# darkAlert/sports-field-homography

Hardware: AMD Instinct MI355X
Metric: frames/sec at 640x360 batch=16 (1/2/4/8 GPU) + homography L1 vs ref (higher is better)
Workload: dtype f16x3->f32 (2-way fp16 split operands = 22 significand bits, 3 fp16 MFMA products, fp32 accumulate; end-to-end error at the level of an fp32 run, see DESIGN.md section 2); 1 GPU; predict(): UNet seg + ResNet34-STN + nearest warp, 640x360, batch 16/GPU, req_outputs=theta,warp_mask; global_batch=16, precision=f16x3, range_fallbacks=0, range_rescales=0, range_raises=0, parallelism=single GPU

## Files before the change

### sports-field-homography_amd/csrc/conv_upfused.hip

```cpp
#include "common.h"
#include "conv_epilogue.h"
#include "split_mfma.h"

namespace {

constexpr int TH = 16, TW = 32;
constexpr int LH = TH / 2 + 2, LW = TW / 2 + 2, LPIX = LH * LW, LPIXP = 192;
constexpr int SHH = TH + 2, SWW = TW + 2, SPIX = SHH * SWW, SPIXP = 624;
constexpr int LSLOTS = 8 * LPIXP, SSLOTS = 8 * SPIXP;

struct UpGeom {
  int tiles_y, tiles_x, ntiles, nblk;
  int xcd_order;
  unsigned bytes_skip, bytes_low;
};

__global__ __launch_bounds__(256, 2) void conv_upfused_kernel(const sfh_conv_desc d, const UpGeom g) {
  extern __shared__ __attribute__((aligned(16))) float smem_f[];
  u32x4* const lds = reinterpret_cast<u32x4*>(smem_f);
  typedef __attribute__((address_space(3))) void* lds_ptr_t;
  const int tid = threadIdx.x, lane = tid & 63, wv = __builtin_amdgcn_readfirstlane(tid >> 6);
  const int lq = lane & 15, lg = lane >> 4;
  const int py = wv >> 1, px = wv & 1, qd = wv;
  int nb, tile;
  if (g.xcd_order) {
    const SfhWg wg = sfh_wg_xcd_range_all((int)blockIdx.x & 7, (int)blockIdx.x >> 3, g.ntiles, g.nblk);
    if (!wg.live) return;
    nb = wg.nb;
    tile = wg.tile;
  } else {
    nb = (int)blockIdx.x % g.nblk;
    tile = (int)blockIdx.x / g.nblk;
  }
  const int tpi = g.tiles_y * g.tiles_x;
  const int b = tile / tpi, tr = tile - b * tpi;
  const int ty = tr / g.tiles_x;
  const int y0 = ty * TH, x0 = (tr - ty * g.tiles_x) * TW;
  const int Y0 = y0 >> 1, X0 = x0 >> 1;
  const int nst_low = d.c1 >> 5, nst_skip = d.c0 >> 5;
  const unsigned nblk_low = (unsigned)d.cs1 >> 5, nblk_skip = (unsigned)d.cs0 >> 5;
  const __amdgpu_buffer_rsrc_t r_skip = __builtin_amdgcn_make_buffer_rsrc(const_cast<float*>(d.src0), 0, (int)g.bytes_skip, 0x00020000);
  const __amdgpu_buffer_rsrc_t r_low = __builtin_amdgcn_make_buffer_rsrc(const_cast<float*>(d.src1), 0, (int)g.bytes_low, 0x00020000);
  using WS = SplitWeights<2>;
  const unsigned wtot_up = (unsigned)nst_low * 4u * WS::TAP, wtot_sk = (unsigned)nst_skip * 9u * WS::TAP;
  const __amdgpu_buffer_rsrc_t rw_up = __builtin_amdgcn_make_buffer_rsrc(
      const_cast<char*>(reinterpret_cast<const char*>(d.up_wpacked)) + (size_t)(qd * g.nblk + nb) * wtot_up, 0, (int)wtot_up, 0x00020000);
  const __amdgpu_buffer_rsrc_t rw_sk = __builtin_amdgcn_make_buffer_rsrc(
      const_cast<char*>(reinterpret_cast<const char*>(d.wpacked)) + (size_t)nb * wtot_sk, 0, (int)wtot_sk, 0x00020000);

  f32x4 acc[4][8];
#pragma unroll
  for (int n = 0; n < 4; ++n)
#pragma unroll
    for (int i = 0; i < 8; ++i) acc[n][i] = (f32x4){0.f, 0.f, 0.f, 0.f};

  auto run_phase = [&](auto ntap_tag, int nst, const __amdgpu_buffer_rsrc_t& rsrc, const __amdgpu_buffer_rsrc_t& rw,
                       auto&& halo_off, int nslots, int rowstride_bytes, auto&& xaddr) {
    constexpr int NTAP = decltype(ntap_tag)::value;
    constexpr int NSTEP = NTAP * 8;
    for (int st = 0; st < nst; ++st) {
      __syncthreads();
      const unsigned cb = (unsigned)st * (unsigned)rowstride_bytes;
      for (int s0 = tid; s0 < nslots; s0 += 256)
        __builtin_amdgcn_raw_ptr_buffer_load_lds(rsrc, (lds_ptr_t)(lds + (s0 - lane)), 16, (int)halo_off(s0), (int)cb, 0, 0);
      u32x4 wr[2][2][4], xq[3][2];
      auto ld_w = [&](int t, int set) {
#pragma unroll
        for (int p = 0; p < 2; ++p)
#pragma unroll
          for (int n = 0; n < 4; ++n)
            wr[set][p][n] = __builtin_bit_cast(u32x4, __builtin_amdgcn_raw_buffer_load_b128(
                rw, (int)((p * 4 + n) * WS::GROUP + lane * 16), (int)(((unsigned)st * NTAP + (unsigned)t) * WS::TAP), 0));
      };
      ld_w(0, 0);
      asm volatile("s_waitcnt vmcnt(8)" ::: "memory");
      __syncthreads();
      auto ld_x = [&](int s_, int set) {
        const int t = s_ >> 3, i = s_ & 7;
#pragma unroll
        for (int p = 0; p < 2; ++p) xq[set][p] = lds[xaddr(t, i, p)];
      };
      ld_x(0, 0);
      ld_x(1, 1);
#pragma unroll
      for (int s_ = 0; s_ < NSTEP; ++s_) {
        const int t = s_ >> 3, i = s_ & 7;
        if (s_ + 2 < NSTEP) ld_x(s_ + 2, (s_ + 2) % 3);
        if (i == 0 && t + 1 < NTAP) ld_w(t + 1, (t + 1) & 1);
        using P = SplitProducts<2>;
#pragma unroll
        for (int k = 0; k < P::N; ++k)
#pragma unroll
          for (int n = 0; n < 4; ++n) acc[n][i] = split_mfma<2>(wr[t & 1][P::PW[k]][n], xq[s_ % 3][P::PX[k]], acc[n][i]);
        __builtin_amdgcn_sched_group_barrier(0x008, 1, 0);
        if (s_ + 2 < NSTEP) __builtin_amdgcn_sched_group_barrier(0x100, 2, 0);
        if (i == 0 && t + 1 < NTAP) __builtin_amdgcn_sched_group_barrier(0x020, 8, 0);
        __builtin_amdgcn_sched_group_barrier(0x008, 11, 0);
        __builtin_amdgcn_sched_barrier(0);
      }
    }
  };

  {
    auto halo_off = [&](int slot) -> unsigned {
      const int plg = slot / LPIXP, p = slot - plg * LPIXP;
      const int hy = p / LW, hx = p - hy * LW;
      const int y = Y0 - 1 + hy, x = X0 - 1 + hx;
      const bool ok = p < LPIX && y >= 0 && y < d.h1 && x >= 0 && x < d.w1;
      return ok ? split_pixel_offset<2>((unsigned)(b * d.h1 + y), nblk_low, (unsigned)plg, (unsigned)d.w1, (unsigned)x) : kSfhOOB;
    };
    const int base = lg * LPIXP + py * LW + lq + px;
    auto xaddr = [&](int t, int i, int p) { return base + p * 4 * LPIXP + (i + (t >> 1)) * LW + (t & 1); };
    run_phase(std::integral_constant<int, 4>{}, nst_low, r_low, rw_up, halo_off, LSLOTS, 128 * d.w1, xaddr);
  }
  const int xo = x0 + 2 * lq + px;
  {
    const int uh = 2 * d.h1, uw = 2 * d.w1;
    const unsigned clsx = (unsigned)(xo == 0 ? 0 : (xo == uw - 1 ? 2 : (xo >= uw ? 3 : 1)));
#pragma unroll
    for (int i = 0; i < 8; ++i) {
      const int yo = y0 + 2 * i + py;
      const unsigned cls = (unsigned)(yo == 0 ? 0 : (yo == uh - 1 ? 2 : (yo >= uh ? 3 : 1))) * 4u + clsx;
#pragma unroll
      for (int n = 0; n < 4; ++n) {
        const int cov = qd * d.cout + nb * 64 + n * 16 + 4 * lg;
        const f32x4 sc = *reinterpret_cast<const f32x4*>(d.up_scale + cov);
        const f32x4 sh = *reinterpret_cast<const f32x4*>(d.shift_border + (size_t)cls * (size_t)(4 * d.cout) + cov);
#pragma unroll
        for (int j = 0; j < 4; ++j) acc[n][i][j] = acc[n][i][j] * sc[j] + sh[j];
      }
    }
  }
  {
    auto halo_off = [&](int slot) -> unsigned {
      const int plg = slot / SPIXP, p = slot - plg * SPIXP;
      const int hy = p / SWW, hx = p - hy * SWW;
      const int y = y0 - 1 + hy, x = x0 - 1 + hx;
      const bool ok = p < SPIX && y >= 0 && y < d.H && x >= 0 && x < d.W;
      return ok ? split_pixel_offset<2>((unsigned)(b * d.H + y), nblk_skip, (unsigned)plg, (unsigned)d.W, (unsigned)x) : kSfhOOB;
    };
    const int base = lg * SPIXP + py * SWW + 2 * lq + px;
    auto xaddr = [&](int t, int i, int p) { return base + p * 4 * SPIXP + (2 * i + t / 3) * SWW + (t % 3); };
    run_phase(std::integral_constant<int, 9>{}, nst_skip, r_skip, rw_sk, halo_off, SSLOTS, 128 * d.W, xaddr);
  }
  const float dscale = sfh_h2_pow2(d.h2_exp_dst);
  const unsigned cs = (unsigned)d.dst_cs, run = (unsigned)d.W * 16u, planeb = 4u * run;
  const __amdgpu_buffer_rsrc_t rd = __builtin_amdgcn_make_buffer_rsrc(d.dst, 0, (int)kSfhOOB, 0x00020000);
  unsigned over = 0u;
#pragma unroll
  for (int n = 0; n < 4; ++n) {
    const unsigned co = (unsigned)(nb * 64 + n * 16 + 4 * lg);
    const f32x4 sc = *reinterpret_cast<const f32x4*>(d.scale + co), sh = *reinterpret_cast<const f32x4*>(d.shift + co);
    const unsigned lane_co = ((co >> 5) * 8u + ((co & 31u) >> 3)) * run + ((co >> 2) & 1u) * 8u;
#pragma unroll
    for (int i = 0; i < 8; ++i) {
      f32x4 v = acc[n][i];
#pragma unroll
      for (int j = 0; j < 4; ++j) {
        v[j] = v[j] * sc[j] + sh[j];
        if (d.relu) v[j] = sfh_relu(v[j]);
      }
      const int yo = y0 + 2 * i + py;
      const bool ok = yo < d.H && xo < d.W;
      const unsigned voff = ok ? (unsigned)(b * d.H + yo) * ((cs >> 5) * 8u * run) + (unsigned)xo * 16u + lane_co : kSfhOOB;
      u32x2 pl[2];
      unsigned o = 0u;
      sfh_split4_h2(v, dscale, pl, o);
      o = ok ? o : 0u;
      over = o > over ? o : over;
#pragma unroll
      for (int p = 0; p < 2; ++p) __builtin_amdgcn_raw_buffer_store_b64(pl[p], rd, (int)voff, (int)(p * planeb), 0);
    }
  }
  sfh_h2_report(over, d.h2_overflow, d.h2_range);
}

}

extern "C" int sfh_conv_upfused_fwd(const sfh_conv_desc* dp, void* stream_) {
  SFH_REQUIRE(dp, "conv_upfused_fwd: null descriptor");
  const sfh_conv_desc& d = *dp;
  SFH_REQUIRE(d.src0 && d.src1 && d.wpacked && d.up_wpacked && d.up_scale && d.shift_border && d.scale && d.shift && d.dst,
              "conv_upfused_fwd: null pointer");
  SFH_REQUIRE(d.src_fmt == SFH_FMT_H2 && d.dst_fmt == SFH_FMT_H2, "conv_upfused_fwd: H2 sources and destination");
  SFH_REQUIRE(d.batch > 0 && d.H > 0 && d.W > 0 && d.h0 == d.H && d.w0 == d.W && d.h1 > 0 && d.w1 > 0 &&
                  (d.H == 2 * d.h1 || d.H == 2 * d.h1 + 1) && (d.W == 2 * d.w1 || d.W == 2 * d.w1 + 1),
              "conv_upfused_fwd: skip %dx%d against a low-resolution source %dx%d (twice its size, plus at most one padded row / column)",
              d.W, d.H, d.w1, d.h1);
  SFH_REQUIRE(d.cout > 0 && d.cout % 64 == 0 && d.c0 > 0 && d.c0 % 32 == 0 && d.cs0 >= d.c0 && d.cs0 % 32 == 0 && d.c1 > 0 &&
                  d.c1 % 32 == 0 && d.cs1 >= d.c1 && d.cs1 % 32 == 0 && d.dst_cs >= d.cout && d.dst_cs % 32 == 0,
              "conv_upfused_fwd: channel counts (cout %d, skip %d / %d, low %d / %d, dst %d)", d.cout, d.c0, d.cs0, d.c1, d.cs1, d.dst_cs);
  SFH_REQUIRE(!d.residual && !d.dst_pool && !d.head_w && !d.acc_init && !(d.ksplit > 1) && !d.stats_partial && !d.pool0,
              "conv_upfused_fwd: a plain launch (no residual / pooled output / head / acc_init / split-K / statistics)");
  if (!sfh_h2_exp_ok("conv_upfused_fwd", "h2_exp_dst", d.h2_exp_dst)) return SFH_E_ARG;
  UpGeom g;
  g.tiles_y = sfh_cdiv(d.H, TH);
  g.tiles_x = sfh_cdiv(d.W, TW);
  g.ntiles = d.batch * g.tiles_y * g.tiles_x;
  g.nblk = d.cout / 64;
  const unsigned long long bs = 4ULL * d.batch * d.H * d.W * d.cs0, bl = 4ULL * d.batch * d.h1 * d.w1 * d.cs1;
  SFH_REQUIRE(sfh_fits_descriptor(bs) && sfh_fits_descriptor(bl) && sfh_fits_descriptor(4ULL * d.batch * d.H * d.W * (unsigned long long)d.dst_cs),
              "conv_upfused_fwd: a tensor exceeds the 4 GiB descriptor range");
  g.bytes_skip = (unsigned)bs;
  g.bytes_low = (unsigned)bl;
  g.xcd_order = 1;
  const long nblocks = (long)sfh_cdiv(g.ntiles, 8) * 8 * g.nblk;
  SFH_REQUIRE(nblocks < (1L << 31), "conv_upfused_fwd: grid too large");
  sfh_allow_big_lds((const void*)conv_upfused_kernel);
  hipLaunchKernelGGL(conv_upfused_kernel, dim3((unsigned)nblocks), dim3(256), SSLOTS * 16, (hipStream_t)stream_, d, g);
  return sfh_check_launch("conv_upfused_kernel");
}
```

Measured before the change: 1275 frames/s.

## Tile upfused conv over batch-flattened rows with incremental halo address walk

Replaces per-image tiling with a grid that treats the batch as one stack of rows, so tiles can span image boundaries and fewer partial tiles are wasted at image edges. The halo staging loop now uses an incremental walker that advances coordinates per round instead of doing divisions per slot, and issues both split planes per iteration. The h2 range report is done with a wave-level max reduction and a single atomic per wave, skipping the atomic when the value is not above a pre-read range. This adds row-split logic per output row and depends on the new shared geometry helpers being correct.

```diff
diff --git a/sports-field-homography_amd/csrc/conv_upfused.hip b/sports-field-homography_amd/csrc/conv_upfused.hip
--- a/sports-field-homography_amd/csrc/conv_upfused.hip
+++ b/sports-field-homography_amd/csrc/conv_upfused.hip
@@ -1,16 +1,14 @@
 #include "common.h"
 #include "conv_epilogue.h"
 #include "split_mfma.h"
+#include "upfused_geom.h"
 
 namespace {
 
-constexpr int TH = 16, TW = 32;
-constexpr int LH = TH / 2 + 2, LW = TW / 2 + 2, LPIX = LH * LW, LPIXP = 192;
-constexpr int SHH = TH + 2, SWW = TW + 2, SPIX = SHH * SWW, SPIXP = 624;
-constexpr int LSLOTS = 8 * LPIXP, SSLOTS = 8 * SPIXP;
-
-struct UpGeom {
-  int tiles_y, tiles_x, ntiles, nblk;
+constexpr int LW = SfhUp::LW, LPIXP = SfhUp::LPIXP, SWW = SfhUp::SWW, SPIXP = SfhUp::SPIXP, SSLOTS = SfhUp::SSLOTS;
+
+struct UpGeom : SfhUpGrid {
+  int nblk;
   int xcd_order;
   unsigned bytes_skip, bytes_low;
 };
@@ -32,13 +30,10 @@
     nb = (int)blockIdx.x % g.nblk;
     tile = (int)blockIdx.x / g.nblk;
   }
-  const int tpi = g.tiles_y * g.tiles_x;
-  const int b = tile / tpi, tr = tile - b * tpi;
-  const int ty = tr / g.tiles_x;
-  const int y0 = ty * TH, x0 = (tr - ty * g.tiles_x) * TW;
-  const int Y0 = y0 >> 1, X0 = x0 >> 1;
+  int r0, x0;
+  sfh_up_tile_origin(g, tile, r0, x0);
+  const SfhUpSrc src_low{d.batch, d.h1, d.w1, (unsigned)d.cs1 >> 5}, src_skip{d.batch, d.H, d.W, (unsigned)d.cs0 >> 5};
   const int nst_low = d.c1 >> 5, nst_skip = d.c0 >> 5;
-  const unsigned nblk_low = (unsigned)d.cs1 >> 5, nblk_skip = (unsigned)d.cs0 >> 5;
   const __amdgpu_buffer_rsrc_t r_skip = __builtin_amdgcn_make_buffer_rsrc(const_cast<float*>(d.src0), 0, (int)g.bytes_skip, 0x00020000);
   const __amdgpu_buffer_rsrc_t r_low = __builtin_amdgcn_make_buffer_rsrc(const_cast<float*>(d.src1), 0, (int)g.bytes_low, 0x00020000);
   using WS = SplitWeights<2>;
@@ -54,15 +49,29 @@
 #pragma unroll
     for (int i = 0; i < 8; ++i) acc[n][i] = (f32x4){0.f, 0.f, 0.f, 0.f};
 
-  auto run_phase = [&](auto ntap_tag, int nst, const __amdgpu_buffer_rsrc_t& rsrc, const __amdgpu_buffer_rsrc_t& rw,
-                       auto&& halo_off, int nslots, int rowstride_bytes, auto&& xaddr) {
+  auto run_phase = [&](auto ntap_tag, auto walk_tag, auto low_tag, int nst, const __amdgpu_buffer_rsrc_t& rsrc,
+                       const __amdgpu_buffer_rsrc_t& rw, const SfhUpSrc& src, int rbase, int xbase, int rowstride_bytes,
+                       auto&& xaddr, auto&& before_last) {
     constexpr int NTAP = decltype(ntap_tag)::value;
     constexpr int NSTEP = NTAP * 8;
+    using Walk = decltype(walk_tag);
     for (int st = 0; st < nst; ++st) {
       __syncthreads();
+      if (st == nst - 1) before_last();
       const unsigned cb = (unsigned)st * (unsigned)rowstride_bytes;
-      for (int s0 = tid; s0 < nslots; s0 += 256)
-        __builtin_amdgcn_raw_ptr_buffer_load_lds(rsrc, (lds_ptr_t)(lds + (s0 - lane)), 16, (int)halo_off(s0), (int)cb, 0, 0);
+      Walk walk;
+      walk.start(tid);
+#pragma unroll 1
+      for (int k = 0; k < Walk::NROUND; ++k) {
+        const int w0 = k * SfhUp::NT + wv * 64;
+        const SfhUpOffsets off = sfh_up_halo_offsets<decltype(low_tag)::value>(g, src, rbase, xbase, walk);
+        if (w0 < Walk::PSLOTS) {
+#pragma unroll
+          for (int p = 0; p < 2; ++p)
+            __builtin_amdgcn_raw_ptr_buffer_load_lds(rsrc, (lds_ptr_t)(lds + (w0 + p * Walk::PSLOTS)), 16, (int)off.plane[p], (int)cb, 0, 0);
+        }
+        walk.step();
+      }
       u32x4 wr[2][2][4], xq[3][2];
       auto ld_w = [&](int t, int set) {
 #pragma unroll
@@ -102,25 +111,19 @@
   };
 
   {
-    auto halo_off = [&](int slot) -> unsigned {
-      const int plg = slot / LPIXP, p = slot - plg * LPIXP;
-      const int hy = p / LW, hx = p - hy * LW;
-      const int y = Y0 - 1 + hy, x = X0 - 1 + hx;
-      const bool ok = p < LPIX && y >= 0 && y < d.h1 && x >= 0 && x < d.w1;
-      return ok ? split_pixel_offset<2>((unsigned)(b * d.h1 + y), nblk_low, (unsigned)plg, (unsigned)d.w1, (unsigned)x) : kSfhOOB;
-    };
     const int base = lg * LPIXP + py * LW + lq + px;
     auto xaddr = [&](int t, int i, int p) { return base + p * 4 * LPIXP + (i + (t >> 1)) * LW + (t & 1); };
-    run_phase(std::integral_constant<int, 4>{}, nst_low, r_low, rw_up, halo_off, LSLOTS, 128 * d.w1, xaddr);
+    run_phase(std::integral_constant<int, 4>{}, SfhUpLowWalk{}, std::true_type{}, nst_low, r_low, rw_up, src_low,
+              sfh_up_low_row(r0) - 1, (x0 >> 1) - 1, 128 * d.w1, xaddr, [] {});
   }
   const int xo = x0 + 2 * lq + px;
   {
-    const int uh = 2 * d.h1, uw = 2 * d.w1;
-    const unsigned clsx = (unsigned)(xo == 0 ? 0 : (xo == uw - 1 ? 2 : (xo >= uw ? 3 : 1)));
+    const unsigned clsx = sfh_up_border_class(xo, 2 * d.w1);
 #pragma unroll
     for (int i = 0; i < 8; ++i) {
-      const int yo = y0 + 2 * i + py;
-      const unsigned cls = (unsigned)(yo == 0 ? 0 : (yo == uh - 1 ? 2 : (yo >= uh ? 3 : 1))) * 4u + clsx;
+      int ob, oy;
+      sfh_row_split(g, r0 + 2 * i + py, ob, oy);
+      const unsigned cls = sfh_up_border_class(oy, 2 * d.h1) * 4u + clsx;
 #pragma unroll
       for (int n = 0; n < 4; ++n) {
         const int cov = qd * d.cout + nb * 64 + n * 16 + 4 * lg;
@@ -131,17 +134,14 @@
       }
     }
   }
+  unsigned range_seen = 0u;
   {
-    auto halo_off = [&](int slot) -> unsigned {
-      const int plg = slot / SPIXP, p = slot - plg * SPIXP;
-      const int hy = p / SWW, hx = p - hy * SWW;
-      const int y = y0 - 1 + hy, x = x0 - 1 + hx;
-      const bool ok = p < SPIX && y >= 0 && y < d.H && x >= 0 && x < d.W;
-      return ok ? split_pixel_offset<2>((unsigned)(b * d.H + y), nblk_skip, (unsigned)plg, (unsigned)d.W, (unsigned)x) : kSfhOOB;
-    };
     const int base = lg * SPIXP + py * SWW + 2 * lq + px;
     auto xaddr = [&](int t, int i, int p) { return base + p * 4 * SPIXP + (2 * i + t / 3) * SWW + (t % 3); };
-    run_phase(std::integral_constant<int, 9>{}, nst_skip, r_skip, rw_sk, halo_off, SSLOTS, 128 * d.W, xaddr);
+    run_phase(std::integral_constant<int, 9>{}, SfhUpSkipWalk{}, std::false_type{}, nst_skip, r_skip, rw_sk, src_skip, r0 - 1,
+              x0 - 1, 128 * d.W, xaddr, [&] {
+                if (d.h2_range) range_seen = *d.h2_range;
+              });
   }
   const float dscale = sfh_h2_pow2(d.h2_exp_dst);
   const unsigned cs = (unsigned)d.dst_cs, run = (unsigned)d.W * 16u, planeb = 4u * run;
@@ -160,9 +160,9 @@
         v[j] = v[j] * sc[j] + sh[j];
         if (d.relu) v[j] = sfh_relu(v[j]);
       }
-      const int yo = y0 + 2 * i + py;
-      const bool ok = yo < d.H && xo < d.W;
-      const unsigned voff = ok ? (unsigned)(b * d.H + yo) * ((cs >> 5) * 8u * run) + (unsigned)xo * 16u + lane_co : kSfhOOB;
+      int ob, oy;
+      const bool ok = sfh_row_split(g, r0 + 2 * i + py, ob, oy, xo < d.W);
+      const unsigned voff = ok ? (unsigned)(ob * d.H + oy) * ((cs >> 5) * 8u * run) + (unsigned)xo * 16u + lane_co : kSfhOOB;
       u32x2 pl[2];
       unsigned o = 0u;
       sfh_split4_h2(v, dscale, pl, o);
@@ -172,7 +172,16 @@
       for (int p = 0; p < 2; ++p) __builtin_amdgcn_raw_buffer_store_b64(pl[p], rd, (int)voff, (int)(p * planeb), 0);
     }
   }
-  sfh_h2_report(over, d.h2_overflow, d.h2_range);
+  if (!d.h2_overflow && !d.h2_range) return;
+#pragma unroll
+  for (int m = 32; m >= 1; m >>= 1) {
+    const unsigned o = (unsigned)__shfl_xor((int)over, m);
+    over = o > over ? o : over;
+  }
+  if (lane == 0) {
+    if (d.h2_overflow && sfh_h2_out_of_range(over)) atomicOr(d.h2_overflow, 1u);
+    if (d.h2_range && over > range_seen) atomicMax(d.h2_range, over);
+  }
 }
 
 }
@@ -194,9 +203,7 @@
               "conv_upfused_fwd: a plain launch (no residual / pooled output / head / acc_init / split-K / statistics)");
   if (!sfh_h2_exp_ok("conv_upfused_fwd", "h2_exp_dst", d.h2_exp_dst)) return SFH_E_ARG;
   UpGeom g;
-  g.tiles_y = sfh_cdiv(d.H, TH);
-  g.tiles_x = sfh_cdiv(d.W, TW);
-  g.ntiles = d.batch * g.tiles_y * g.tiles_x;
+  SFH_REQUIRE(sfh_up_grid(g, d.batch, d.H, d.W), "conv_upfused_fwd: too many rows");
   g.nblk = d.cout / 64;
   const unsigned long long bs = 4ULL * d.batch * d.H * d.W * d.cs0, bl = 4ULL * d.batch * d.h1 * d.w1 * d.cs1;
   SFH_REQUIRE(sfh_fits_descriptor(bs) && sfh_fits_descriptor(bl) && sfh_fits_descriptor(4ULL * d.batch * d.H * d.W * (unsigned long long)d.dst_cs),
diff --git a/sports-field-homography_amd/csrc/upfused_geom.h b/sports-field-homography_amd/csrc/upfused_geom.h
--- /dev/null
+++ b/sports-field-homography_amd/csrc/upfused_geom.h
@@ -0,0 +1,91 @@
+#pragma once
+#include "conv_geom.h"
+
+struct SfhUp {
+  static constexpr int NT = 256;
+  static constexpr int TH = 16, TW = 32;
+  static constexpr int LH = TH / 2 + 2, LW = TW / 2 + 2, LPIX = LH * LW, LPIXP = 192;
+  static constexpr int SHH = TH + 2, SWW = TW + 2, SPIX = SHH * SWW, SPIXP = 624;
+  static constexpr int LSLOTS = 8 * LPIXP, SSLOTS = 8 * SPIXP;
+};
+
+struct SfhUpGrid {
+  int tiles_x, tiles_y, ntiles;
+  int Ho, Wo, rows_total, rows_per_img;
+  unsigned rows_magic;
+};
+
+SFH_GEOM_FN bool sfh_up_grid(SfhUpGrid& g, int batch, int H, int W) {
+  return sfh_conv_grid(g, batch, H, W, 3, 1, true, true, SfhUp::TH, SfhUp::TW);
+}
+
+SFH_GEOM_FN void sfh_up_tile_origin(const SfhUpGrid& g, int tile, int& r0, int& x0) {
+  const int ty = tile / g.tiles_x;
+  r0 = ty * SfhUp::TH;
+  x0 = (tile - ty * g.tiles_x) * SfhUp::TW;
+}
+
+SFH_GEOM_FN int sfh_up_low_row(int r) { return r >> 1; }
+
+template <bool LOW>
+SFH_GEOM_FN void sfh_up_row_split(const SfhUpGrid& g, int r, int& b, int& y) {
+  sfh_row_split(g, LOW ? 2 * r : r, b, y);
+  if (LOW) y = r - b * (g.rows_per_img >> 1);
+}
+
+SFH_GEOM_FN unsigned sfh_up_border_class(int v, int n) { return v == 0 ? 0u : (v == n - 1 ? 2u : (v >= n ? 3u : 1u)); }
+
+template <int HW_, int HPIX_, int HPIXP_>
+struct SfhUpHaloWalk {
+  static constexpr int HW = HW_, HPIX = HPIX_, HPIXP = HPIXP_, PSLOTS = 4 * HPIXP;
+  static constexpr int NROUND = (PSLOTS + SfhUp::NT - 1) / SfhUp::NT;
+  static_assert(PSLOTS % 64 == 0, "whole waves");
+  static constexpr int QP = SfhUp::NT / HPIXP, RP = SfhUp::NT % HPIXP;
+  static constexpr int QH = RP / HW, RH = RP % HW;
+  static constexpr int QX = HPIXP / HW, RX = HPIXP % HW;
+  int plg, p, hy, hx;
+  SFH_GEOM_FN void start(int tid) {
+    plg = tid / HPIXP;
+    p = tid - plg * HPIXP;
+    hy = p / HW;
+    hx = p - hy * HW;
+  }
+  SFH_GEOM_FN void step() {
+    plg += QP;
+    p += RP;
+    hy += QH;
+    hx += RH;
+    const bool cx = hx >= HW;
+    hx -= cx ? HW : 0;
+    hy += cx ? 1 : 0;
+    const bool cp = p >= HPIXP;
+    p -= cp ? HPIXP : 0;
+    plg += cp ? 1 : 0;
+    hy -= cp ? QX : 0;
+    hx -= cp ? RX : 0;
+    const bool cb = hx < 0;
+    hx += cb ? HW : 0;
+    hy -= cb ? 1 : 0;
+  }
+};
+using SfhUpLowWalk = SfhUpHaloWalk<SfhUp::LW, SfhUp::LPIX, SfhUp::LPIXP>;
+using SfhUpSkipWalk = SfhUpHaloWalk<SfhUp::SWW, SfhUp::SPIX, SfhUp::SPIXP>;
+
+struct SfhUpSrc {
+  int batch, h, w;
+  unsigned nblk;
+};
+
+struct SfhUpOffsets {
+  unsigned plane[2];
+};
+template <bool LOW, class Walk>
+SFH_GEOM_FN SfhUpOffsets sfh_up_halo_offsets(const SfhUpGrid& g, const SfhUpSrc& s, int rbase, int xbase, const Walk& w) {
+  const int r = rbase + w.hy, x = xbase + w.hx;
+  int b, y;
+  sfh_up_row_split<LOW>(g, r < 0 ? 0 : r, b, y);
+  const bool ok = (w.p < Walk::HPIX) & (r >= 0) & (b < s.batch) & (y < s.h) & ((unsigned)x < (unsigned)s.w);
+  const unsigned run = (unsigned)s.w * 16u;
+  const unsigned off = ((unsigned)(b * s.h + y) * (s.nblk * 8u) + (unsigned)w.plg) * run + (unsigned)x * 16u;
+  return SfhUpOffsets{{ok ? off : kSfhOOB, ok ? off + 4u * run : kSfhOOB}};
+}
```

Measured after the change: 1285 frames/s (median of 6 runs). No clear change (+0.7%).
